# scitix/arks

Hardware: AMD Instinct MI355X
Metric: output_tok_s (higher is better)
Workload: dtype bf16; 1 GPU; model=qwen2.5-7b, global_batch=64, seq_len=1024, parallelism=dp1

## Files before the change

arks_amd/ops/__init__.py:

```python

from __future__ import annotations

import os
from typing import Callable, NamedTuple

import torch

from . import ref

_C = None
_C_ERR: str | None = None


def _load_extension():
    global _C, _C_ERR
    if _C is not None or _C_ERR is not None:
        return _C
    try:
        from . import _load

        _C = _load.C
    except Exception as e:
        _C_ERR = f"{type(e).__name__}: {e}"
    return _C
# ... 59 lines not shown
                   cos_sin, head_dim: int):
    if q.is_cuda:
        _native().rope_and_cache(positions, q, k, v, k_cache, v_cache,
                                 slot_mapping, cos_sin, head_dim)
        return q, k
    q2, k2 = ref.rope_apply(positions, q, k, cos_sin, head_dim)
    T = q.shape[0]
    nkv = k.numel() // max(T, 1) // head_dim
    ref.reshape_and_cache(
        k2.reshape(T, nkv, head_dim), v.reshape(T, nkv, head_dim),
        k_cache, v_cache, slot_mapping,
    )
    return q2, k2


def rope_and_cache_splitk(positions, qkv, k_cache, v_cache, slot_mapping,
                          cos_sin, head_dim: int, num_q_heads: int):
    qkv.check_live()
    if qkv.shape[1] != (num_q_heads + 2 * k_cache.shape[1]) * head_dim:
        raise ValueError(f"qkv width {qkv.shape[1]} does not match the heads")
    q = torch.empty((qkv.shape[0], num_q_heads * head_dim),
                    dtype=torch.bfloat16, device=qkv.ws.device)
    _native().splitk_rope_and_cache(positions, qkv.ws, qkv.bias, q, k_cache,
                                    v_cache, slot_mapping, cos_sin, head_dim,
                                    qkv.nsplits, qkv.mrows)
    return q


def reshape_and_cache(k, v, k_cache, v_cache, slot_mapping):
    if k.is_cuda:
        _native().reshape_and_cache(k, v, k_cache, v_cache, slot_mapping)
        return
    ref.reshape_and_cache(k, v, k_cache, v_cache, slot_mapping)


PREFILL_QTILE = 64


def build_prefill_tiles(seq_lens: list[int], device) -> torch.Tensor:
    tiles = []
# ... 207 lines not shown

    def materialize(self) -> torch.Tensor:
        self.check_live()
        out = torch.empty(self.shape, dtype=torch.bfloat16,
                          device=self.ws.device)
        _native().skinny_combine(out, self.ws, self.bias, self.nsplits,
                                 self.mrows)
        return out


def skinny_gemm(x, weight, bias=None, defer: bool = False):
    M, K = x.shape
    N = weight.shape[0]
    config, nsplits, k_per_split, mrows = _skinny_plan(M, N, K)
    config = _skinny_resident_config(config, M, nsplits, k_per_split)
    part = (_skinny_ws(nsplits, N, mrows, x.device) if nsplits > 1
            else x.new_empty(0, dtype=torch.float32))
    if defer and nsplits > 1:
        _native().skinny_gemm_partials(part, x, weight, k_per_split, nsplits,
                                       config)
        return SplitKPending(part, nsplits, mrows, M, N, bias,
                             (x.device.index,))
    out = torch.empty((M, N), dtype=x.dtype, device=x.device)
    _native().skinny_gemm(out, part, x, weight, bias, k_per_split, nsplits,
                          config)
    return out


def _skinny_plan(M: int, N: int, K: int):
    ntiles = N // 64
# ... 7 lines not shown
    nsplits = -(-K // k_per_split)
    return config, nsplits, k_per_split, 16 * mt


_SKINNY_RESIDENT_KMAX = 512
_SKINNY_RESIDENT = os.environ.get("ARKS_SKINNY_RESIDENT", "1") == "1"
_SKINNY_RESIDENT_MIN_M = 1


def _skinny_resident_config(config: int, M: int, nsplits: int,
                            k_per_split: int) -> int:
    if (_SKINNY_RESIDENT and config == 0 and nsplits > 1
            and k_per_split <= _SKINNY_RESIDENT_KMAX
            and M >= _SKINNY_RESIDENT_MIN_M):
        return 3
    return config


def _skinny_ws(nsplits: int, N: int, mrows: int, device):
    key = (device.index,)
    need = nsplits * N * mrows
    ws = _SKINNY_WS.get(key)
    if ws is None or ws.numel() < need:
        ws = torch.empty(need, dtype=torch.float32, device=device)
        _SKINNY_WS[key] = ws
    _SKINNY_WS_GEN[key] = _SKINNY_WS_GEN.get(key, 0) + 1
    return ws


_USE_SKINNY = os.environ.get("ARKS_SKINNY_GEMM", "1") == "1"
# ... 300 lines not shown
        out = torch.empty(T, H, dtype=y.dtype, device=y.device)
        _native().moe_mix(out, y.contiguous(), weights, ids, expert_base, El)
        return out
    return ref.moe_mix(y, weights, ids, expert_base)


def moe_mix_rows(y, weights, rows):
    if y.is_cuda:
        T, k = weights.shape
        out = torch.empty(T, y.shape[1], dtype=y.dtype, device=y.device)
        _native().moe_mix_rows(out, y.contiguous(), weights, rows)
        return out
    return ref.moe_mix_rows(y, weights, rows)


def sample_tokens(logits, temperatures, uniform):
    if logits.is_cuda:
        out = torch.empty(logits.shape[0], dtype=torch.int64, device=logits.device)
        _native().gumbel_sample(out, logits, temperatures, uniform)
        return out
    return ref.gumbel_sample(logits, temperatures, uniform)


def greedy_sample(logits):
    if logits.is_cuda:
        out = torch.empty(logits.shape[0], dtype=torch.int64, device=logits.device)
        _native().greedy_sample(out, logits)
        return out
    return ref.greedy_sample(logits)


def greedy_sample_masked(logits, masks, mask_row):
    if logits.is_cuda:
        out = torch.empty(logits.shape[0], dtype=torch.int64, device=logits.device)
        _native().greedy_sample_masked(out, logits, masks, mask_row)
        return out
    return ref.greedy_sample_masked(logits, masks, mask_row)


def sample_tokens_masked(logits, temperatures, uniform, masks, mask_row):
    if logits.is_cuda:
        out = torch.empty(logits.shape[0], dtype=torch.int64, device=logits.device)
        _native().gumbel_sample_masked(out, logits, temperatures, uniform,
# ... 114 lines not shown
```

arks_amd/ops/csrc/bindings.cpp:

```cpp
#include <torch/extension.h>

#include <c10/hip/HIPStream.h>
#include <hip/hip_runtime.h>

#include <cstring>
#include <string>
#include <vector>

namespace py = pybind11;

extern "C" {
void arks_rmsnorm(void* out, const void* input, const void* weight, float eps,
                  int rows, int hidden, hipStream_t stream);
void arks_fused_add_rmsnorm(void* out, const void* input, void* residual,
                            const void* weight, float eps, int rows, int hidden,
                            hipStream_t stream);
void arks_silu_mul(void* out, const void* gate_up, int64_t rows, int d,
                   hipStream_t stream);
int arks_pool_max_hidden();
void arks_pool_embed(void* out, void* carry, void* part, const void* x,
                     const void* residual, const void* weight,
                     const void* segs, const void* slabs, int nsegs,
                     int nslabs, float eps, int hidden, int dims,
                     int normalize, hipStream_t stream);
// ... 59 lines not shown
int arks_skinny_slab_rows(int m_rows, int config);
int arks_skinny_resident_kmax();
void arks_skinny_combine(void* out, const void* part, const void* bias,
                         int m_rows, int n_total, int nsplits, int mrows_pad,
                         hipStream_t stream);
void arks_splitk_add_rmsnorm(void* out, const void* part, const void* bias,
                             void* residual, const void* weight, float eps,
                             int rows, int hidden, int nsplits, int mrows_pad,
                             hipStream_t stream);
void arks_splitk_rope_and_cache(const void* positions, const void* part,
                                const void* bias, void* q_out, void* k_cache,
                                void* v_cache, const void* slot_mapping,
                                const void* cos_sin, int num_tokens,
                                int head_dim, int num_q_heads,
                                int num_kv_heads, int block_size, int nsplits,
                                int mrows_pad, int kv_fp8, hipStream_t stream);
void arks_greedy_sample(void* out, const void* logits, int rows, int vocab,
                        hipStream_t stream);
void arks_gumbel_sample(void* out, const void* logits, const void* temperatures,
                        const void* uniform, int rows, int vocab,
                        hipStream_t stream);
void arks_greedy_sample_masked(void* out, const void* logits,
                               const void* masks, const void* mask_row,
                               int rows, int vocab, int slots,
                               hipStream_t stream);
void arks_gumbel_sample_masked(void* out, const void* logits,
                               const void* temperatures, const void* uniform,
                               const void* masks, const void* mask_row,
                               int rows, int vocab, int slots,
                               hipStream_t stream);
void arks_apply_token_bitmask(void* logits, int is_fp32, const void* masks,
                              const void* mask_row, int rows, int vocab,
                              int slots, hipStream_t stream);
void arks_ar_seq_inc(void* seq, hipStream_t stream);
void arks_one_shot_allreduce(void* out, const void* src, void* mail_ptrs[8],
                             void* flag_ptrs[8], void* seq, int rank,
// ... 301 lines not shown
  TORCH_CHECK(combine_table.scalar_type() == torch::kInt32 &&
              combine_table.dim() == 2 && combine_table.size(1) == 4);
  const int num_q_heads = out.size(1);
  const int head_dim = out.size(2);
  arks_attn_extend2_combine(out.data_ptr(), part_ws.data_ptr(),
                            combine_table.data_ptr(), cu_seqlens_q.data_ptr(),
                            combine_table.size(0), (float)scale, num_q_heads,
                            head_dim, current_stream());
}

const void* check_skinny_args(const torch::Tensor& out,
                              const torch::Tensor& part,
                              const torch::Tensor& a, const torch::Tensor& w,
                              const c10::optional<torch::Tensor>& bias,
                              int64_t k, int64_t nsplits, int64_t mrows,
                              bool partials_only, const char* what) {
  check_bf16_rowstrided(a, "a");
  check_bf16_contig(w, "w");
  const int64_t m = a.size(0), n = w.size(0);
  TORCH_CHECK(m >= 1 && m <= 64, what, " needs 1 <= M <= 64");
  TORCH_CHECK(n % 64 == 0 && k % 32 == 0, "N%64==0 and K%32==0 required");
  if (partials_only) {
    TORCH_CHECK(nsplits > 1, what, ": partials-only needs nsplits > 1");
  } else {
    check_bf16_contig(out, "out");
    TORCH_CHECK(out.size(0) == m && out.size(1) == n);
  }
  const void* bias_ptr = nullptr;
  if (bias.has_value()) {
    check_bf16_contig(*bias, "bias");
    TORCH_CHECK(bias->numel() == n);
    bias_ptr = bias->data_ptr();
  }
  if (nsplits > 1) {
    TORCH_CHECK(part.is_cuda() && part.scalar_type() == torch::kFloat32 &&
                part.is_contiguous() &&
                part.numel() >= (int64_t)nsplits * n * mrows,
                what, " workspace too small");
  }
  return bias_ptr;
}

void skinny_gemm_impl(torch::Tensor out, torch::Tensor part, torch::Tensor a,
                      torch::Tensor w, c10::optional<torch::Tensor> bias,
                      int64_t k_per_split, int64_t nsplits, int64_t config,
                      int64_t groups, bool combine) {
  const int m = a.size(0), k = a.size(1), n = w.size(0);
  TORCH_CHECK(w.size(1) == k);
  TORCH_CHECK(0 <= config && config <= 3, "config in 0..3");
  TORCH_CHECK(k_per_split >= 32 && k_per_split % 32 == 0 &&
              nsplits * k_per_split >= k, "splits must cover K");
  TORCH_CHECK(config != 3 ||
                  (nsplits > 1 && k_per_split <= arks_skinny_resident_kmax()),
              "config 3 needs nsplits > 1 and k_per_split <= ",
              arks_skinny_resident_kmax());
  TORCH_CHECK(0 <= groups && groups <= 65535, "groups in 0..65535");
  TORCH_CHECK(nsplits <= 65535, "too many splits");
  const int mrows = arks_skinny_slab_rows(m, (int)config);
  const void* bias_ptr = check_skinny_args(out, part, a, w, bias, k, nsplits,
                                           mrows, !combine, "skinny_gemm");
  arks_skinny_gemm(nsplits > 1 ? part.data_ptr() : nullptr,
                   combine ? out.data_ptr() : nullptr, a.data_ptr(),
                   w.data_ptr(), bias_ptr, m, n, k, (int)k_per_split,
                   (int)nsplits, a.stride(0), (int)config, combine,
                   current_stream(), (int)groups);
}

void skinny_gemm(torch::Tensor out, torch::Tensor part, torch::Tensor a,
                 torch::Tensor w, c10::optional<torch::Tensor> bias,
                 int64_t k_per_split, int64_t nsplits, int64_t config,
                 int64_t groups) {
  skinny_gemm_impl(out, part, a, w, bias, k_per_split, nsplits, config, groups,
                   true);
}

// ... 277 lines not shown
              weight.numel() == hidden);
  const void* bias_ptr = check_partials(part, bias, nsplits, mrows, rows,
                                        hidden);
  if (rows == 0) return;
  arks_splitk_add_rmsnorm(out.data_ptr(), part.data_ptr(), bias_ptr,
                          residual.data_ptr(), weight.data_ptr(), (float)eps,
                          rows, hidden, (int)nsplits, (int)mrows,
                          current_stream());
}

void splitk_rope_and_cache(torch::Tensor positions, torch::Tensor part,
                           c10::optional<torch::Tensor> bias,
                           torch::Tensor q_out, torch::Tensor k_cache,
                           torch::Tensor v_cache, torch::Tensor slot_mapping,
                           torch::Tensor cos_sin, int64_t head_dim,
                           int64_t nsplits, int64_t mrows) {
  TORCH_CHECK(positions.scalar_type() == torch::kInt64 &&
              positions.is_contiguous());
  TORCH_CHECK(slot_mapping.scalar_type() == torch::kInt64 &&
              slot_mapping.is_contiguous());
  TORCH_CHECK(cos_sin.scalar_type() == torch::kFloat32 &&
              cos_sin.is_contiguous() && cos_sin.size(-1) == head_dim);
  check_bf16_contig(q_out, "q_out");
  const bool kv_fp8 = check_kv_cache(k_cache, "k_cache");
  TORCH_CHECK(check_kv_cache(v_cache, "v_cache") == kv_fp8);
  TORCH_CHECK(q_out.dim() == 2 && head_dim % 8 == 0);
  const int T = q_out.size(0);
  const int nq = (int)(q_out.size(1) / head_dim);
  const int nkv = k_cache.size(1);
  const int block_size = k_cache.size(2);
  TORCH_CHECK(nq * head_dim == q_out.size(1) && k_cache.size(3) == head_dim &&
              v_cache.sizes() == k_cache.sizes());
  TORCH_CHECK(positions.numel() == T && slot_mapping.numel() == T);
  const void* bias_ptr = check_partials(part, bias, nsplits, mrows, T,
                                        (int64_t)(nq + 2 * nkv) * head_dim);
  arks_splitk_rope_and_cache(positions.data_ptr(), part.data_ptr(), bias_ptr,
                             q_out.data_ptr(), k_cache.data_ptr(),
                             v_cache.data_ptr(), slot_mapping.data_ptr(),
                             cos_sin.data_ptr(), T, (int)head_dim, nq, nkv,
                             block_size, (int)nsplits, (int)mrows,
                             kv_fp8 ? 1 : 0, current_stream());
}

void rmsnorm_fp8(torch::Tensor out, torch::Tensor inv_scale,
                 torch::Tensor input, c10::optional<torch::Tensor> residual,
                 torch::Tensor weight, double eps) {
  check_bf16_contig(input, "input");
  check_bf16_contig(weight, "weight");
  TORCH_CHECK(out.scalar_type() == torch::kFloat8_e4m3fn && out.is_contiguous());
  TORCH_CHECK(inv_scale.scalar_type() == torch::kFloat32);
  const int hidden = input.size(-1);
  TORCH_CHECK(hidden % 8 == 0 && hidden <= 8192,
              "rmsnorm_fp8 requires hidden % 8 == 0 and hidden <= 8192");
  const int rows = input.numel() / hidden;
  void* res_ptr = nullptr;
  if (residual.has_value()) {
// ... 16 lines not shown
  const int rows = out.numel() / d;
  arks_silu_mul_fp8(out.data_ptr(), inv_scale.data_ptr(), gate_up.data_ptr(),
                    rows, d, current_stream());
}

void quant_fp8_rows(torch::Tensor out, torch::Tensor inv_scale,
                    torch::Tensor x) {
  check_bf16_contig(x, "x");
  TORCH_CHECK(out.scalar_type() == torch::kFloat8_e4m3fn && out.is_contiguous());
  TORCH_CHECK(inv_scale.scalar_type() == torch::kFloat32);
  TORCH_CHECK(x.size(1) % 8 == 0, "cols must be a multiple of 8");
  arks_quant_fp8_rows(out.data_ptr(), inv_scale.data_ptr(), x.data_ptr(),
                      x.size(0), x.size(1), current_stream());
}

void greedy_sample(torch::Tensor out, torch::Tensor logits) {
  check_bf16_contig(logits, "logits");
  TORCH_CHECK(out.scalar_type() == torch::kInt64);
  arks_greedy_sample(out.data_ptr(), logits.data_ptr(), logits.size(0),
                     logits.size(1), current_stream());
}

void gumbel_sample(torch::Tensor out, torch::Tensor logits,
                   torch::Tensor temperatures, torch::Tensor uniform) {
  check_bf16_contig(logits, "logits");
  TORCH_CHECK(out.scalar_type() == torch::kInt64);
  TORCH_CHECK(temperatures.scalar_type() == torch::kFloat32);
  TORCH_CHECK(uniform.scalar_type() == torch::kFloat32);
  arks_gumbel_sample(out.data_ptr(), logits.data_ptr(), temperatures.data_ptr(),
                     uniform.data_ptr(), logits.size(0), logits.size(1),
                     current_stream());
}

static void check_bitmask(const torch::Tensor& logits,
                          const torch::Tensor& masks,
                          const torch::Tensor& mask_row) {
  TORCH_CHECK(logits.dim() == 2 && masks.dim() == 2 && mask_row.dim() == 1);
  TORCH_CHECK(masks.is_cuda() && mask_row.is_cuda());
  TORCH_CHECK(masks.scalar_type() == torch::kInt32 && masks.is_contiguous());
  TORCH_CHECK(mask_row.scalar_type() == torch::kInt32 &&
              mask_row.is_contiguous());
  TORCH_CHECK(masks.size(1) == (logits.size(1) + 31) / 32,
              "masks must have ceil(vocab/32) words per row");
  TORCH_CHECK(mask_row.size(0) == logits.size(0), "one mask_row per row");
}
// ... 335 lines not shown
  m.def("skinny_gemm", &skinny_gemm, py::arg("out"), py::arg("part"),
        py::arg("a"), py::arg("w"), py::arg("bias"), py::arg("k_per_split"),
        py::arg("nsplits"), py::arg("config") = 0, py::arg("groups") = 0);
  m.def("skinny_gemm_partials", &skinny_gemm_partials, py::arg("part"),
        py::arg("a"), py::arg("w"), py::arg("k_per_split"),
        py::arg("nsplits"), py::arg("config") = 0, py::arg("groups") = 0);
  m.def("skinny_combine", &skinny_combine);
  m.def("w4_skinny_gemm", &w4_skinny_gemm);
  m.def("w4_skinny_gemm_partials", &w4_skinny_gemm_partials);
  m.def("w4_dequant", &w4_dequant);
  m.def("w4_moe_gemm", &w4_moe_gemm);
  m.def("w8_skinny_gemm", &w8_skinny_gemm);
  m.def("w8_skinny_gemm_partials", &w8_skinny_gemm_partials);
  m.def("w8_dequant", &w8_dequant);
  m.def("splitk_add_rmsnorm", &splitk_add_rmsnorm);
  m.def("splitk_rope_and_cache", &splitk_rope_and_cache);
  m.def("greedy_sample", &greedy_sample);
  m.def("gumbel_sample", &gumbel_sample);
  m.def("greedy_sample_masked", &greedy_sample_masked);
  m.def("gumbel_sample_masked", &gumbel_sample_masked);
  m.def("apply_token_bitmask", &apply_token_bitmask);
  m.def("ipc_alloc", &ipc_alloc);
  m.def("arm_flags", &arm_flags);
  m.def("ipc_alloc_free", &ipc_alloc_free);
  m.def("ipc_handle", &ipc_handle);
  m.def("ipc_open", &ipc_open);
  m.def("ipc_close", &ipc_close);
  m.def("one_shot_allreduce", &one_shot_allreduce);
  m.def("moe_topk", &moe_topk);
  m.def("moe_route", &moe_route);
  m.def("moe_mix", &moe_mix);
  m.def("moe_mix_rows", &moe_mix_rows);
  m.def("lora_shrink", &lora_shrink);
// ... 7 lines not shown
```

arks_amd/ops/csrc/kvcache.hip:

```cpp
#include "kv_store.h"

#include <type_traits>

namespace arks {

template <bool FP8>
__global__ void reshape_and_cache_kernel(
    const bf16* __restrict__ k,
    const bf16* __restrict__ v,
    void* __restrict__ k_cache,
    void* __restrict__ v_cache,
    const int64_t* __restrict__ slot_mapping,
    const int num_kv_heads, const int head_dim, const int block_size,
    const int64_t kv_stride) {
  const int token = blockIdx.x;
  const CachePage pg =
      cache_page(slot_mapping[token], num_kv_heads, block_size, head_dim);
  if (!pg.valid) return;
  const int nvec = num_kv_heads * head_dim / 8;
  const bf16* k_src = k + (int64_t)token * kv_stride;
  const bf16* v_src = v + (int64_t)token * kv_stride;
  for (int i = threadIdx.x; i < nvec; i += blockDim.x) {
    const int h = (i * 8) / head_dim;
    const int d = (i * 8) % head_dim;
// ... 78 lines not shown
    const int block_size, const int nsplits, const int64_t split_stride) {
  const int token = blockIdx.x;
  const int half = head_dim / 2;
  const int n_total = (num_q_heads + 2 * num_kv_heads) * head_dim;
  const int64_t pos = positions[token];
  const float* cs = cos_sin + pos * head_dim;
  const CachePage pg =
      cache_page(slot_mapping[token], num_kv_heads, block_size, head_dim);
  const float* part_row = part + (int64_t)token * n_total;

  const int quads = half / 4;
  const int nrot_q = num_q_heads * quads;
  const int nrot = pg.valid ? nrot_q + num_kv_heads * quads : nrot_q;
  const int nvec = pg.valid ? num_kv_heads * head_dim / 8 : 0;
  const int v_col0 = (num_q_heads + num_kv_heads) * head_dim;
  for (int idx = threadIdx.x; idx < nrot + nvec; idx += blockDim.x) {
    if (idx < nrot) {
      const int h = idx / quads;
      const int p4 = (idx % quads) * 4;
      const int col = h * head_dim + p4;
      const float* const p[2] = {part_row + col, part_row + col + half};
      float4v acc[2];
      splitk_reduce<2, 1>(p, split_stride, nsplits, acc);
      ushort4v o1, o2;
#pragma unroll
      for (int j = 0; j < 4; ++j) {
        float af = acc[0][j];
        float bf = acc[1][j];
        if (bias != nullptr) {
          af += bf16_bits_to_float(bias[col + j]);
          bf += bf16_bits_to_float(bias[col + half + j]);
// ... 56 lines not shown
  int threads = std::min(256, num_kv_heads * head_dim / 8);
  dispatch_kv_fp8(kv_fp8, [&](auto fp8) {
    hipLaunchKernelGGL((reshape_and_cache_kernel<decltype(fp8)::value>),
                       dim3(num_tokens), dim3(threads), 0, stream,
                       (const bf16*)k, (const bf16*)v, k_cache, v_cache,
                       (const int64_t*)slot_mapping, num_kv_heads, head_dim,
                       block_size, kv_stride);
  });
}

extern "C" void arks_splitk_rope_and_cache(
    const void* positions, const void* part, const void* bias, void* q_out,
    void* k_cache, void* v_cache, const void* slot_mapping,
    const void* cos_sin, int num_tokens, int head_dim, int num_q_heads,
    int num_kv_heads, int block_size, int nsplits, int mrows_pad, int kv_fp8,
    hipStream_t stream) {
  if (num_tokens == 0) return;
  const int items = (num_q_heads + num_kv_heads) * (head_dim / 8) +
                    num_kv_heads * head_dim / 8;
  dim3 grid(num_tokens), block(std::min(1024, (items + 63) / 64 * 64));
  const int64_t split_stride =
      (int64_t)mrows_pad * (num_q_heads + 2 * num_kv_heads) * head_dim;
  dispatch_kv_fp8(kv_fp8, [&](auto fp8) {
    hipLaunchKernelGGL((splitk_rope_cache_kernel<decltype(fp8)::value>), grid,
                       block, 0, stream, (const int64_t*)positions,
                       (const float*)part, (const bf16*)bias, (bf16*)q_out,
                       k_cache, v_cache, (const int64_t*)slot_mapping,
                       (const float*)cos_sin, head_dim, num_q_heads,
                       num_kv_heads, block_size, nsplits, split_stride);
  });
}

extern "C" void arks_rope_and_cache(
    const void* positions, void* q, void* k, const void* v, void* k_cache,
    void* v_cache, const void* slot_mapping, const void* cos_sin,
// ... 15 lines not shown
```

arks_amd/ops/csrc/sampling.hip:

```cpp
#include "common.h"

#include <cfloat>

namespace arks {

template <bool GUMBEL>
__global__ void sample_kernel(int64_t* __restrict__ out,
                              const bf16* __restrict__ logits,
                              const float* __restrict__ temperatures,
                              const float* __restrict__ uniform,
                              const int vocab) {
  constexpr int BLOCK = 256;
  const int row = blockIdx.x;
  const bf16* lrow = logits + (int64_t)row * vocab;
  float inv_t = 0.f;
  bool greedy = true;
  if constexpr (GUMBEL) {
    const float t = temperatures[row];
    greedy = (t <= 0.f);
    inv_t = greedy ? 1.f : 1.f / t;
  }
  const float* urow = GUMBEL ? uniform + (int64_t)row * vocab : nullptr;

  float best = -FLT_MAX;
  int best_idx = 0;
  const int nvec = vocab / 8;
  for (int i = threadIdx.x; i < nvec; i += BLOCK) {
    ushort8 x = *reinterpret_cast<const ushort8*>(lrow + i * 8);
#pragma unroll
    for (int j = 0; j < 8; ++j) {
      float v = bf16_bits_to_float(x[j]);
      if constexpr (GUMBEL) {
        if (!greedy) {
          float u = urow[i * 8 + j];
          u = fmaxf(u, 1e-20f);
          v = v * inv_t - __logf(-__logf(u));
        }
      }
      const int idx = i * 8 + j;
      if (v > best || (v == best && idx < best_idx)) {
        best = v;
        best_idx = idx;
      }
    }
  }
  for (int idx = nvec * 8 + threadIdx.x; idx < vocab; idx += BLOCK) {
    float v = bf16_bits_to_float(lrow[idx]);
    if constexpr (GUMBEL) {
      if (!greedy) {
        float u = fmaxf(urow[idx], 1e-20f);
        v = v * inv_t - __logf(-__logf(u));
      }
    }
    if (v > best || (v == best && idx < best_idx)) {
      best = v;
      best_idx = idx;
    }
  }

#pragma unroll
  for (int off = 32; off > 0; off >>= 1) {
    float ov = __shfl_xor(best, off, WAVE_SIZE);
    int oi = __shfl_xor(best_idx, off, WAVE_SIZE);
    if (ov > best || (ov == best && oi < best_idx)) {
      best = ov;
      best_idx = oi;
    }
  }
  __shared__ float sval[BLOCK / WAVE_SIZE];
  __shared__ int sidx[BLOCK / WAVE_SIZE];
  const int wave = threadIdx.x / WAVE_SIZE;
  if (threadIdx.x % WAVE_SIZE == 0) {
    sval[wave] = best;
    sidx[wave] = best_idx;
  }
  __syncthreads();
  if (threadIdx.x == 0) {
    float b = sval[0];
    int bi = sidx[0];
#pragma unroll
    for (int w = 1; w < BLOCK / WAVE_SIZE; ++w) {
      if (sval[w] > b || (sval[w] == b && sidx[w] < bi)) {
        b = sval[w];
        bi = sidx[w];
      }
    }
    out[row] = bi;
  }
}

constexpr int NO_TOKEN = 0x7fffffff;

__device__ __forceinline__ void masked_take(float v, int idx, float& best,
                                            int& best_idx, bool allowed = true) {
  const bool take =
      allowed & ((v > best) | ((v == best) & (idx < best_idx)));
  best = take ? v : best;
  best_idx = take ? idx : best_idx;
}

template <bool GUMBEL>
__global__ void sample_masked_kernel(int64_t* __restrict__ out,
                                     const bf16* __restrict__ logits,
// ... 115 lines not shown
  if (idx0 >= vocab) return;
  const uint32_t word = masks[(int64_t)mr * words + (idx0 >> 5)];
  const uint32_t bits = (word >> (idx0 & 31)) & 0xffu;
  if (bits == 0xffu) return;
  T* lrow = logits + (int64_t)row * vocab;
#pragma unroll
  for (int j = 0; j < 8; ++j) {
    if (idx0 + j < vocab && !((bits >> j) & 1u)) lrow[idx0 + j] = neg_inf;
  }
}

}

using namespace arks;

extern "C" {

void arks_greedy_sample_masked(void* out, const void* logits,
                               const void* masks, const void* mask_row,
                               int rows, int vocab, int slots,
                               hipStream_t stream) {
  hipLaunchKernelGGL((sample_masked_kernel<false>), dim3(rows), dim3(256), 0,
                     stream, (int64_t*)out, (const bf16*)logits, nullptr,
                     nullptr, (const uint32_t*)masks, (const int*)mask_row,
                     vocab, (vocab + 31) / 32, slots);
}

void arks_gumbel_sample_masked(void* out, const void* logits,
                               const void* temperatures, const void* uniform,
                               const void* masks, const void* mask_row,
// ... 11 lines not shown
                              int slots, hipStream_t stream) {
  const dim3 grid(rows, (vocab + 2047) / 2048);
  const int words = (vocab + 31) / 32;
  if (is_fp32) {
    hipLaunchKernelGGL((apply_bitmask_kernel<float>), grid, dim3(256), 0,
                       stream, (float*)logits, (const uint32_t*)masks,
                       (const int*)mask_row, vocab, words, slots, -INFINITY);
  } else {
    hipLaunchKernelGGL((apply_bitmask_kernel<uint16_t>), grid, dim3(256), 0,
                       stream, (uint16_t*)logits, (const uint32_t*)masks,
                       (const int*)mask_row, vocab, words, slots,
                       (uint16_t)0xff80);
  }
}

void arks_greedy_sample(void* out, const void* logits, int rows, int vocab,
                        hipStream_t stream) {
  hipLaunchKernelGGL((sample_kernel<false>), dim3(rows), dim3(256), 0, stream,
                     (int64_t*)out, (const bf16*)logits, nullptr, nullptr,
                     vocab);
}

void arks_gumbel_sample(void* out, const void* logits, const void* temperatures,
                        const void* uniform, int rows, int vocab,
                        hipStream_t stream) {
  hipLaunchKernelGGL((sample_kernel<true>), dim3(rows), dim3(256), 0, stream,
                     (int64_t*)out, (const bf16*)logits,
                     (const float*)temperatures, (const float*)uniform, vocab);
}

}
```

arks_amd/ops/csrc/skinny_gemm.hip:

```cpp
#include "common.h"

#include <algorithm>
#include <atomic>
#include <cfloat>
#include <type_traits>

namespace arks {

typedef __attribute__((ext_vector_type(8))) __bf16 bf16x8;
typedef __attribute__((ext_vector_type(4))) float f32x4;

__device__ __forceinline__ f32x4 sk_mfma(bf16x8 a, bf16x8 b, f32x4 c) {
  return __builtin_amdgcn_mfma_f32_16x16x32_bf16(a, b, c, 0, 0, 0);
}

constexpr int SK_AP = 8;

template <int MT>
__device__ __forceinline__ void store_partials(float* __restrict__ part,
                                               const f32x4 (&acc)[MT],
                                               const int n_total,
                                               const int n, const int lq) {
  float* p = part + (int64_t)blockIdx.y * (16 * MT) * n_total + n;
#pragma unroll
// ... 8 lines not shown
__global__ __launch_bounds__(64 * WAVES, 2) void skinny_gemm_kernel(
    float* __restrict__ part,
    bf16* __restrict__ out,
    const bf16* __restrict__ a,
    const bf16* __restrict__ w,
    const bf16* __restrict__ bias,
    const int m_rows, const int n_total, const int k_total,
    const int k_per_split, const int nsplits, const int64_t a_stride) {
  constexpr int KC = SK_KC;
  constexpr int D = SK_D;
  constexpr int KSTEPS = KC / 32;
  constexpr int CPT = KC / 8;
  constexpr int THREADS = 64 * WAVES;
  constexpr int NTW = 16 * WAVES;
  constexpr int RPP = THREADS / CPT;
  constexpr int NIT = 16 * MT / RPP;
  static_assert(D % 2 == 0, "LDS slot parity follows the ring slot");
  static_assert(NIT * RPP == 16 * MT, "A chunk must divide over the threads");
  const int n0 = blockIdx.x * NTW;
  const int kb = blockIdx.y * k_per_split;
  const int ke = min(k_total, kb + k_per_split);
  const int klen = max(ke - kb, 0);
  const int nch = (klen + KC - 1) / KC;

  const int tid = threadIdx.x;
  const int wave = tid / WAVE_SIZE;
  const int lane = tid % WAVE_SIZE;
  const int lq = lane % 16;
  const int la = lane / 16;

  __shared__ __attribute__((aligned(16))) union {
    bf16 a_buf[2][64][KC + SK_AP];
    float c_buf[NTW][64 + 1];
// ... 25 lines not shown
      ad[it] = *reinterpret_cast<const ushort8*>(live ? src : a);
    }
#pragma unroll
    for (int s = 0; s < KSTEPS; ++s) {
      const bf16* wsrc = wrow + min(kc + s * 32, k_total - 32);
      const ushort8* src =
          reinterpret_cast<const ushort8*>(live ? wsrc : w);
      if constexpr (NT)
        wd[s] = __builtin_nontemporal_load(src);
      else
        wd[s] = *src;
    }
  };
  auto write_a = [&](const ushort8 (&ad)[NIT], int buf) {
#pragma unroll
    for (int it = 0; it < NIT; ++it)
      *reinterpret_cast<ushort8*>(
          &lds.a_buf[buf][tid / CPT + it * RPP][acol]) = ad[it];
  };
  auto mfma_chunk = [&](const ushort8 (&wd)[KSTEPS], int buf, int kw) {
#pragma unroll
    for (int s = 0; s < KSTEPS; ++s) {
      if (s * 32 >= kw) break;
      ushort8 wv = wd[s];
      bf16x8 wfrag = *reinterpret_cast<bf16x8*>(&wv);
#pragma unroll
      for (int t = 0; t < MT; ++t) {
        ushort8 af = *reinterpret_cast<const ushort8*>(
            &lds.a_buf[buf][t * 16 + lq][s * 32 + 8 * la]);
        acc[t] = sk_mfma(wfrag, *reinterpret_cast<bf16x8*>(&af), acc[t]);
      }
    }
  };
// ... 315 lines not shown
      launch_resident<decltype(mt)::value>(
          (float*)part, (const bf16*)a, (const bf16*)w, m_rows, n_total,
          k_total, k_per_split, nsplits, a_stride, groups, stream);
    };
    switch (skinny_mt(m_rows, config)) {
      case 1: launch(std::integral_constant<int, 1>{}); break;
      case 2: launch(std::integral_constant<int, 2>{}); break;
      case 3: launch(std::integral_constant<int, 3>{}); break;
      default: launch(std::integral_constant<int, 4>{}); break;
    }
    if (combine)
      arks_skinny_combine(out, part, bias, m_rows, n_total, nsplits,
                          arks_skinny_slab_rows(m_rows, config), stream);
    return;
  }
  const int waves = config == 0 ? 4 : 8;
  dim3 grid((n_total + 16 * waves - 1) / (16 * waves), nsplits);
  dim3 block(64 * waves);
  auto launch = [&](auto kernel) {
    hipLaunchKernelGGL(kernel, grid, block, 0, stream, (float*)part,
                       (bf16*)out, (const bf16*)a, (const bf16*)w,
                       (const bf16*)bias, m_rows, n_total, k_total,
                       k_per_split, nsplits, a_stride);
  };
  if (config == 2) {
    launch(skinny_gemm_kernel<4, true, 8>);
  } else if (config == 1) {
    launch(skinny_gemm_kernel<4, false, 8>);
  } else {
    switch (skinny_mt(m_rows, config)) {
      case 1: launch(skinny_gemm_kernel<1>); break;
      case 2: launch(skinny_gemm_kernel<2>); break;
      case 3: launch(skinny_gemm_kernel<3>); break;
      default: launch(skinny_gemm_kernel<4>); break;
    }
  }
  if (nsplits > 1 && combine)
    arks_skinny_combine(out, part, bias, m_rows, n_total, nsplits,
                        arks_skinny_slab_rows(m_rows, config), stream);
}
// ... 1 lines not shown
```

Before: 12140 tok/s.

## Split sampling, rope-cache and tall-K skinny GEMM across more workgroups

Adds a chunked two-pass argmax sampler that splits each vocab row over several workgroups when rows are fewer than CUs, then merges per-chunk pairs. Also splits the split-K rope/KV-cache kernel over a second grid dimension sized from the CU count. Adds a 7-wave (112-column) tall-K skinny GEMM variant, chosen when it fills more CUs without exceeding them. The aim is better CU occupancy for small-batch decode, at the cost of an extra merge launch and workspace allocation.

```diff
diff --git a/arks_amd/ops/__init__.py b/arks_amd/ops/__init__.py
--- a/arks_amd/ops/__init__.py
+++ b/arks_amd/ops/__init__.py
@@ -97,16 +97,28 @@
     return q2, k2
 
 
+_ROPE_SPLITK_GROUPS = int(os.environ.get("ARKS_ROPE_SPLITK_GROUPS", "0"))
+
+
+def _rope_splitk_groups(tokens: int, cus: int) -> int:
+    if _ROPE_SPLITK_GROUPS > 0:
+        return _ROPE_SPLITK_GROUPS
+    return max(1, -(-cus // max(tokens, 1)))
+
+
 def rope_and_cache_splitk(positions, qkv, k_cache, v_cache, slot_mapping,
-                          cos_sin, head_dim: int, num_q_heads: int):
+                          cos_sin, head_dim: int, num_q_heads: int,
+                          groups: int | None = None):
     qkv.check_live()
     if qkv.shape[1] != (num_q_heads + 2 * k_cache.shape[1]) * head_dim:
         raise ValueError(f"qkv width {qkv.shape[1]} does not match the heads")
     q = torch.empty((qkv.shape[0], num_q_heads * head_dim),
                     dtype=torch.bfloat16, device=qkv.ws.device)
+    if groups is None:
+        groups = _rope_splitk_groups(qkv.shape[0], _cu_count(qkv.ws.device))
     _native().splitk_rope_and_cache(positions, qkv.ws, qkv.bias, q, k_cache,
                                     v_cache, slot_mapping, cos_sin, head_dim,
-                                    qkv.nsplits, qkv.mrows)
+                                    qkv.nsplits, qkv.mrows, groups)
     return q
 
 
@@ -344,6 +356,9 @@
     N = weight.shape[0]
     config, nsplits, k_per_split, mrows = _skinny_plan(M, N, K)
     config = _skinny_resident_config(config, M, nsplits, k_per_split)
+    if config == 1:
+        config = _skinny_tallk7_config(config, N, nsplits,
+                                       _cu_count(x.device))
     part = (_skinny_ws(nsplits, N, mrows, x.device) if nsplits > 1
             else x.new_empty(0, dtype=torch.float32))
     if defer and nsplits > 1:
@@ -381,6 +396,23 @@
             and k_per_split <= _SKINNY_RESIDENT_KMAX
             and M >= _SKINNY_RESIDENT_MIN_M):
         return 3
+    return config
+
+
+_TALLK_WAVES = os.environ.get("ARKS_SKINNY_TALLK_WAVES", "7").strip()
+if _TALLK_WAVES not in ("7", "8"):
+    raise ValueError(
+        f"ARKS_SKINNY_TALLK_WAVES={_TALLK_WAVES!r}: accepted values are 7 "
+        "(112-row tiles where they fill more CUs) and 8 (128-row tiles)"
+    )
+
+
+def _skinny_tallk7_config(config: int, N: int, nsplits: int, cus: int) -> int:
+    if _TALLK_WAVES != "7" or config != 1 or N % 112 != 0:
+        return config
+    wgs = N // 112 * nsplits
+    if wgs <= cus and wgs > -(-N // 128) * nsplits:
+        return 4
     return config
 
 
@@ -711,19 +743,49 @@
     return ref.moe_mix_rows(y, weights, rows)
 
 
-def sample_tokens(logits, temperatures, uniform):
+_CU_COUNT: dict = {}
+
+
+def _cu_count(device) -> int:
+    idx = device.index if device.index is not None else torch.cuda.current_device()
+    n = _CU_COUNT.get(idx)
+    if n is None:
+        n = _CU_COUNT[idx] = torch.cuda.get_device_properties(idx).multi_processor_count
+    return n
+
+
+_SAMPLE_MIN_CHUNK = 2048
+_SAMPLE_WGS_PER_CU = 4
+
+
+def _sample_chunks(rows: int, vocab: int, cus: int) -> int:
+    if rows >= cus:
+        return 1
+    want = -(-_SAMPLE_WGS_PER_CU * cus // max(rows, 1))
+    return max(1, min(want, vocab // _SAMPLE_MIN_CHUNK))
+
+
+def _sample_launch(fn, logits, args, chunks):
+    rows, vocab = logits.shape
+    if chunks is None:
+        chunks = _sample_chunks(rows, vocab, _cu_count(logits.device))
+    out = torch.empty(rows, dtype=torch.int64, device=logits.device)
+    pairs = (torch.empty((rows, chunks, 2), dtype=torch.int32,
+                         device=logits.device) if chunks > 1 else None)
+    fn(out, logits, *args, pairs, chunks)
+    return out
+
+
+def sample_tokens(logits, temperatures, uniform, chunks=None):
     if logits.is_cuda:
-        out = torch.empty(logits.shape[0], dtype=torch.int64, device=logits.device)
-        _native().gumbel_sample(out, logits, temperatures, uniform)
-        return out
+        return _sample_launch(_native().gumbel_sample, logits,
+                              (temperatures, uniform), chunks)
     return ref.gumbel_sample(logits, temperatures, uniform)
 
 
-def greedy_sample(logits):
+def greedy_sample(logits, chunks=None):
     if logits.is_cuda:
-        out = torch.empty(logits.shape[0], dtype=torch.int64, device=logits.device)
-        _native().greedy_sample(out, logits)
-        return out
+        return _sample_launch(_native().greedy_sample, logits, (), chunks)
     return ref.greedy_sample(logits)
 
 
diff --git a/arks_amd/ops/csrc/bindings.cpp b/arks_amd/ops/csrc/bindings.cpp
--- a/arks_amd/ops/csrc/bindings.cpp
+++ b/arks_amd/ops/csrc/bindings.cpp
@@ -97,12 +97,13 @@
                                 const void* cos_sin, int num_tokens,
                                 int head_dim, int num_q_heads,
                                 int num_kv_heads, int block_size, int nsplits,
-                                int mrows_pad, int kv_fp8, hipStream_t stream);
-void arks_greedy_sample(void* out, const void* logits, int rows, int vocab,
-                        hipStream_t stream);
-void arks_gumbel_sample(void* out, const void* logits, const void* temperatures,
-                        const void* uniform, int rows, int vocab,
-                        hipStream_t stream);
+                                int mrows_pad, int kv_fp8, int groups,
+                                hipStream_t stream);
+void arks_greedy_sample(void* out, void* pairs, const void* logits, int rows,
+                        int vocab, int chunks, hipStream_t stream);
+void arks_gumbel_sample(void* out, void* pairs, const void* logits,
+                        const void* temperatures, const void* uniform,
+                        int rows, int vocab, int chunks, hipStream_t stream);
 void arks_greedy_sample_masked(void* out, const void* logits,
                                const void* masks, const void* mask_row,
                                int rows, int vocab, int slots,
@@ -434,12 +435,14 @@
                               const torch::Tensor& a, const torch::Tensor& w,
                               const c10::optional<torch::Tensor>& bias,
                               int64_t k, int64_t nsplits, int64_t mrows,
-                              bool partials_only, const char* what) {
+                              int64_t n_mult, bool partials_only,
+                              const char* what) {
   check_bf16_rowstrided(a, "a");
   check_bf16_contig(w, "w");
   const int64_t m = a.size(0), n = w.size(0);
   TORCH_CHECK(m >= 1 && m <= 64, what, " needs 1 <= M <= 64");
-  TORCH_CHECK(n % 64 == 0 && k % 32 == 0, "N%64==0 and K%32==0 required");
+  TORCH_CHECK(n % n_mult == 0 && k % 32 == 0, "N%", n_mult,
+              "==0 and K%32==0 required");
   if (partials_only) {
     TORCH_CHECK(nsplits > 1, what, ": partials-only needs nsplits > 1");
   } else {
@@ -467,7 +470,7 @@
                       int64_t groups, bool combine) {
   const int m = a.size(0), k = a.size(1), n = w.size(0);
   TORCH_CHECK(w.size(1) == k);
-  TORCH_CHECK(0 <= config && config <= 3, "config in 0..3");
+  TORCH_CHECK(0 <= config && config <= 4, "config in 0..4");
   TORCH_CHECK(k_per_split >= 32 && k_per_split % 32 == 0 &&
               nsplits * k_per_split >= k, "splits must cover K");
   TORCH_CHECK(config != 3 ||
@@ -477,8 +480,10 @@
   TORCH_CHECK(0 <= groups && groups <= 65535, "groups in 0..65535");
   TORCH_CHECK(nsplits <= 65535, "too many splits");
   const int mrows = arks_skinny_slab_rows(m, (int)config);
-  const void* bias_ptr = check_skinny_args(out, part, a, w, bias, k, nsplits,
-                                           mrows, !combine, "skinny_gemm");
+  const void* bias_ptr =
+      check_skinny_args(out, part, a, w, bias, k, nsplits, mrows,
+                        config == 0 || config == 3 ? 64 : 16, !combine,
+                        "skinny_gemm");
   arks_skinny_gemm(nsplits > 1 ? part.data_ptr() : nullptr,
                    combine ? out.data_ptr() : nullptr, a.data_ptr(),
                    w.data_ptr(), bias_ptr, m, n, k, (int)k_per_split,
@@ -786,7 +791,8 @@
                            torch::Tensor q_out, torch::Tensor k_cache,
                            torch::Tensor v_cache, torch::Tensor slot_mapping,
                            torch::Tensor cos_sin, int64_t head_dim,
-                           int64_t nsplits, int64_t mrows) {
+                           int64_t nsplits, int64_t mrows, int64_t groups) {
+  TORCH_CHECK(1 <= groups && groups <= 65535, "groups in 1..65535");
   TORCH_CHECK(positions.scalar_type() == torch::kInt64 &&
               positions.is_contiguous());
   TORCH_CHECK(slot_mapping.scalar_type() == torch::kInt64 &&
@@ -811,7 +817,7 @@
                              v_cache.data_ptr(), slot_mapping.data_ptr(),
                              cos_sin.data_ptr(), T, (int)head_dim, nq, nkv,
                              block_size, (int)nsplits, (int)mrows,
-                             kv_fp8 ? 1 : 0, current_stream());
+                             kv_fp8 ? 1 : 0, (int)groups, current_stream());
 }
 
 void rmsnorm_fp8(torch::Tensor out, torch::Tensor inv_scale,
@@ -858,21 +864,40 @@
                       x.size(0), x.size(1), current_stream());
 }
 
-void greedy_sample(torch::Tensor out, torch::Tensor logits) {
+static void* check_sample_pairs(const torch::Tensor& out,
+                                const torch::Tensor& logits,
+                                const c10::optional<torch::Tensor>& pairs,
+                                int64_t chunks) {
   check_bf16_contig(logits, "logits");
-  TORCH_CHECK(out.scalar_type() == torch::kInt64);
-  arks_greedy_sample(out.data_ptr(), logits.data_ptr(), logits.size(0),
-                     logits.size(1), current_stream());
+  TORCH_CHECK(logits.dim() == 2);
+  TORCH_CHECK(out.scalar_type() == torch::kInt64 && out.is_contiguous() &&
+              out.numel() >= logits.size(0));
+  TORCH_CHECK(1 <= chunks && chunks <= 65535, "chunks in 1..65535");
+  if (chunks == 1) return nullptr;
+  TORCH_CHECK(pairs.has_value() && pairs->is_cuda() &&
+                  pairs->scalar_type() == torch::kInt32 &&
+                  pairs->is_contiguous() &&
+                  pairs->numel() >= logits.size(0) * chunks * 2,
+              "chunks > 1 needs an int32 workspace of rows * chunks * 2");
+  return pairs->data_ptr();
+}
+
+void greedy_sample(torch::Tensor out, torch::Tensor logits,
+                   c10::optional<torch::Tensor> pairs, int64_t chunks) {
+  void* ws = check_sample_pairs(out, logits, pairs, chunks);
+  arks_greedy_sample(out.data_ptr(), ws, logits.data_ptr(), logits.size(0),
+                     logits.size(1), (int)chunks, current_stream());
 }
 
 void gumbel_sample(torch::Tensor out, torch::Tensor logits,
-                   torch::Tensor temperatures, torch::Tensor uniform) {
-  check_bf16_contig(logits, "logits");
-  TORCH_CHECK(out.scalar_type() == torch::kInt64);
+                   torch::Tensor temperatures, torch::Tensor uniform,
+                   c10::optional<torch::Tensor> pairs, int64_t chunks) {
+  void* ws = check_sample_pairs(out, logits, pairs, chunks);
   TORCH_CHECK(temperatures.scalar_type() == torch::kFloat32);
   TORCH_CHECK(uniform.scalar_type() == torch::kFloat32);
-  arks_gumbel_sample(out.data_ptr(), logits.data_ptr(), temperatures.data_ptr(),
-                     uniform.data_ptr(), logits.size(0), logits.size(1),
+  arks_gumbel_sample(out.data_ptr(), ws, logits.data_ptr(),
+                     temperatures.data_ptr(), uniform.data_ptr(),
+                     logits.size(0), logits.size(1), (int)chunks,
                      current_stream());
 }
 
@@ -1238,9 +1263,16 @@
   m.def("w8_skinny_gemm_partials", &w8_skinny_gemm_partials);
   m.def("w8_dequant", &w8_dequant);
   m.def("splitk_add_rmsnorm", &splitk_add_rmsnorm);
-  m.def("splitk_rope_and_cache", &splitk_rope_and_cache);
-  m.def("greedy_sample", &greedy_sample);
-  m.def("gumbel_sample", &gumbel_sample);
+  m.def("splitk_rope_and_cache", &splitk_rope_and_cache, py::arg("positions"),
+        py::arg("part"), py::arg("bias"), py::arg("q_out"), py::arg("k_cache"),
+        py::arg("v_cache"), py::arg("slot_mapping"), py::arg("cos_sin"),
+        py::arg("head_dim"), py::arg("nsplits"), py::arg("mrows"),
+        py::arg("groups") = 1);
+  m.def("greedy_sample", &greedy_sample, py::arg("out"), py::arg("logits"),
+        py::arg("pairs") = py::none(), py::arg("chunks") = 1);
+  m.def("gumbel_sample", &gumbel_sample, py::arg("out"), py::arg("logits"),
+        py::arg("temperatures"), py::arg("uniform"),
+        py::arg("pairs") = py::none(), py::arg("chunks") = 1);
   m.def("greedy_sample_masked", &greedy_sample_masked);
   m.def("gumbel_sample_masked", &gumbel_sample_masked);
   m.def("apply_token_bitmask", &apply_token_bitmask);
diff --git a/arks_amd/ops/csrc/kvcache.hip b/arks_amd/ops/csrc/kvcache.hip
--- a/arks_amd/ops/csrc/kvcache.hip
+++ b/arks_amd/ops/csrc/kvcache.hip
@@ -116,7 +116,8 @@
   const int nrot = pg.valid ? nrot_q + num_kv_heads * quads : nrot_q;
   const int nvec = pg.valid ? num_kv_heads * head_dim / 8 : 0;
   const int v_col0 = (num_q_heads + num_kv_heads) * head_dim;
-  for (int idx = threadIdx.x; idx < nrot + nvec; idx += blockDim.x) {
+  for (int idx = blockIdx.y * blockDim.x + threadIdx.x; idx < nrot + nvec;
+       idx += blockDim.x * gridDim.y) {
     if (idx < nrot) {
       const int h = idx / quads;
       const int p4 = (idx % quads) * 4;
@@ -203,11 +204,14 @@
     void* k_cache, void* v_cache, const void* slot_mapping,
     const void* cos_sin, int num_tokens, int head_dim, int num_q_heads,
     int num_kv_heads, int block_size, int nsplits, int mrows_pad, int kv_fp8,
-    hipStream_t stream) {
+    int groups, hipStream_t stream) {
   if (num_tokens == 0) return;
   const int items = (num_q_heads + num_kv_heads) * (head_dim / 8) +
                     num_kv_heads * head_dim / 8;
-  dim3 grid(num_tokens), block(std::min(1024, (items + 63) / 64 * 64));
+  groups = std::max(1, std::min(groups, (items + 63) / 64));
+  const int per_group = (items + groups - 1) / groups;
+  dim3 grid(num_tokens, groups);
+  dim3 block(std::min(1024, (per_group + 63) / 64 * 64));
   const int64_t split_stride =
       (int64_t)mrows_pad * (num_q_heads + 2 * num_kv_heads) * head_dim;
   dispatch_kv_fp8(kv_fp8, [&](auto fp8) {
diff --git a/arks_amd/ops/csrc/sampling.hip b/arks_amd/ops/csrc/sampling.hip
--- a/arks_amd/ops/csrc/sampling.hip
+++ b/arks_amd/ops/csrc/sampling.hip
@@ -1,31 +1,33 @@
 #include "common.h"
 
+#include <algorithm>
 #include <cfloat>
 
 namespace arks {
 
+constexpr int SAMPLE_BLOCK = 256;
+
+__device__ __forceinline__ void sample_take(float v, int idx, float& best,
+                                            int& best_idx) {
+  if (v > best || (v == best && idx < best_idx)) {
+    best = v;
+    best_idx = idx;
+  }
+}
+
 template <bool GUMBEL>
-__global__ void sample_kernel(int64_t* __restrict__ out,
-                              const bf16* __restrict__ logits,
-                              const float* __restrict__ temperatures,
-                              const float* __restrict__ uniform,
-                              const int vocab) {
-  constexpr int BLOCK = 256;
-  const int row = blockIdx.x;
-  const bf16* lrow = logits + (int64_t)row * vocab;
-  float inv_t = 0.f;
-  bool greedy = true;
-  if constexpr (GUMBEL) {
-    const float t = temperatures[row];
-    greedy = (t <= 0.f);
-    inv_t = greedy ? 1.f : 1.f / t;
-  }
-  const float* urow = GUMBEL ? uniform + (int64_t)row * vocab : nullptr;
-
-  float best = -FLT_MAX;
-  int best_idx = 0;
-  const int nvec = vocab / 8;
-  for (int i = threadIdx.x; i < nvec; i += BLOCK) {
+__device__ __forceinline__ bool sample_scan(const bf16* __restrict__ lrow,
+                                            const float* __restrict__ urow,
+                                            const bool greedy,
+                                            const float inv_t, const int begin,
+                                            const int end, float& best,
+                                            int& best_idx) {
+  constexpr int BLOCK = SAMPLE_BLOCK;
+  best = -FLT_MAX;
+  best_idx = 0;
+  const int vec0 = begin / 8;
+  const int nvec = end / 8;
+  for (int i = vec0 + threadIdx.x; i < nvec; i += BLOCK) {
     ushort8 x = *reinterpret_cast<const ushort8*>(lrow + i * 8);
 #pragma unroll
     for (int j = 0; j < 8; ++j) {
@@ -37,14 +39,10 @@
           v = v * inv_t - __logf(-__logf(u));
         }
       }
-      const int idx = i * 8 + j;
-      if (v > best || (v == best && idx < best_idx)) {
-        best = v;
-        best_idx = idx;
-      }
-    }
-  }
-  for (int idx = nvec * 8 + threadIdx.x; idx < vocab; idx += BLOCK) {
+      sample_take(v, i * 8 + j, best, best_idx);
+    }
+  }
+  for (int idx = nvec * 8 + threadIdx.x; idx < end; idx += BLOCK) {
     float v = bf16_bits_to_float(lrow[idx]);
     if constexpr (GUMBEL) {
       if (!greedy) {
@@ -52,20 +50,14 @@
         v = v * inv_t - __logf(-__logf(u));
       }
     }
-    if (v > best || (v == best && idx < best_idx)) {
-      best = v;
-      best_idx = idx;
-    }
+    sample_take(v, idx, best, best_idx);
   }
 
 #pragma unroll
   for (int off = 32; off > 0; off >>= 1) {
     float ov = __shfl_xor(best, off, WAVE_SIZE);
     int oi = __shfl_xor(best_idx, off, WAVE_SIZE);
-    if (ov > best || (ov == best && oi < best_idx)) {
-      best = ov;
-      best_idx = oi;
-    }
+    sample_take(ov, oi, best, best_idx);
   }
   __shared__ float sval[BLOCK / WAVE_SIZE];
   __shared__ int sidx[BLOCK / WAVE_SIZE];
@@ -75,18 +67,67 @@
     sidx[wave] = best_idx;
   }
   __syncthreads();
-  if (threadIdx.x == 0) {
-    float b = sval[0];
-    int bi = sidx[0];
-#pragma unroll
-    for (int w = 1; w < BLOCK / WAVE_SIZE; ++w) {
-      if (sval[w] > b || (sval[w] == b && sidx[w] < bi)) {
-        b = sval[w];
-        bi = sidx[w];
-      }
-    }
-    out[row] = bi;
-  }
+  if (threadIdx.x != 0) return false;
+  best = sval[0];
+  best_idx = sidx[0];
+#pragma unroll
+  for (int w = 1; w < BLOCK / WAVE_SIZE; ++w)
+    sample_take(sval[w], sidx[w], best, best_idx);
+  return true;
+}
+
+template <bool GUMBEL>
+__global__ __launch_bounds__(SAMPLE_BLOCK) void sample_kernel(
+    int64_t* __restrict__ out,
+    int2* __restrict__ pairs,
+    const bf16* __restrict__ logits,
+    const float* __restrict__ temperatures,
+    const float* __restrict__ uniform,
+    const int vocab, const int chunk_len) {
+  const int row = blockIdx.x;
+  const bf16* lrow = logits + (int64_t)row * vocab;
+  float inv_t = 0.f;
+  bool greedy = true;
+  if constexpr (GUMBEL) {
+    const float t = temperatures[row];
+    greedy = (t <= 0.f);
+    inv_t = greedy ? 1.f : 1.f / t;
+  }
+  const float* urow = GUMBEL ? uniform + (int64_t)row * vocab : nullptr;
+
+  const int begin =
+      (int)std::min<int64_t>((int64_t)blockIdx.y * chunk_len, vocab);
+  const int end = (int)std::min<int64_t>((int64_t)begin + chunk_len, vocab);
+  float best;
+  int best_idx;
+  if (!sample_scan<GUMBEL>(lrow, urow, greedy, inv_t, begin, end, best,
+                           best_idx))
+    return;
+  if (gridDim.y == 1)
+    out[row] = best_idx;
+  else
+    pairs[(int64_t)row * gridDim.y + blockIdx.y] =
+        make_int2(__float_as_int(best), best_idx);
+}
+
+__global__ __launch_bounds__(64) void sample_merge_kernel(
+    int64_t* __restrict__ out, const int2* __restrict__ pairs, const int rows,
+    const int chunks) {
+  const int row = blockIdx.x * 64 + threadIdx.x;
+  if (row >= rows) return;
+  float best = -FLT_MAX;
+  int best_idx = 0;
+  constexpr int BATCH = 16;
+  const int2* prow = pairs + (int64_t)row * chunks;
+  for (int c = 0; c < chunks; c += BATCH) {
+    int2 p[BATCH];
+#pragma unroll
+    for (int j = 0; j < BATCH; ++j) p[j] = prow[min(c + j, chunks - 1)];
+#pragma unroll
+    for (int j = 0; j < BATCH; ++j)
+      sample_take(__int_as_float(p[j].x), p[j].y, best, best_idx);
+  }
+  out[row] = best_idx;
 }
 
 constexpr int NO_TOKEN = 0x7fffffff;
@@ -232,6 +273,25 @@
 
 using namespace arks;
 
+template <bool GUMBEL>
+static void launch_sample(void* out, void* pairs, const void* logits,
+                          const void* temperatures, const void* uniform,
+                          int rows, int vocab, int chunks,
+                          hipStream_t stream) {
+  chunks = std::max(chunks, 1);
+  const int chunk_len =
+      chunks == 1 ? vocab : ((vocab + chunks - 1) / chunks + 7) / 8 * 8;
+  hipLaunchKernelGGL((sample_kernel<GUMBEL>), dim3(rows, chunks),
+                     dim3(SAMPLE_BLOCK), 0, stream, (int64_t*)out,
+                     (int2*)pairs, (const bf16*)logits,
+                     (const float*)temperatures, (const float*)uniform, vocab,
+                     chunk_len);
+  if (chunks > 1)
+    hipLaunchKernelGGL(sample_merge_kernel, dim3((rows + 63) / 64), dim3(64),
+                       0, stream, (int64_t*)out, (const int2*)pairs, rows,
+                       chunks);
+}
+
 extern "C" {
 
 void arks_greedy_sample_masked(void* out, const void* logits,
@@ -273,19 +333,17 @@
   }
 }
 
-void arks_greedy_sample(void* out, const void* logits, int rows, int vocab,
-                        hipStream_t stream) {
-  hipLaunchKernelGGL((sample_kernel<false>), dim3(rows), dim3(256), 0, stream,
-                     (int64_t*)out, (const bf16*)logits, nullptr, nullptr,
-                     vocab);
-}
-
-void arks_gumbel_sample(void* out, const void* logits, const void* temperatures,
-                        const void* uniform, int rows, int vocab,
-                        hipStream_t stream) {
-  hipLaunchKernelGGL((sample_kernel<true>), dim3(rows), dim3(256), 0, stream,
-                     (int64_t*)out, (const bf16*)logits,
-                     (const float*)temperatures, (const float*)uniform, vocab);
-}
-
-}
+void arks_greedy_sample(void* out, void* pairs, const void* logits, int rows,
+                        int vocab, int chunks, hipStream_t stream) {
+  launch_sample<false>(out, pairs, logits, nullptr, nullptr, rows, vocab,
+                       chunks, stream);
+}
+
+void arks_gumbel_sample(void* out, void* pairs, const void* logits,
+                        const void* temperatures, const void* uniform,
+                        int rows, int vocab, int chunks, hipStream_t stream) {
+  launch_sample<true>(out, pairs, logits, temperatures, uniform, rows, vocab,
+                      chunks, stream);
+}
+
+}
diff --git a/arks_amd/ops/csrc/skinny_gemm.hip b/arks_amd/ops/csrc/skinny_gemm.hip
--- a/arks_amd/ops/csrc/skinny_gemm.hip
+++ b/arks_amd/ops/csrc/skinny_gemm.hip
@@ -46,9 +46,8 @@
   constexpr int THREADS = 64 * WAVES;
   constexpr int NTW = 16 * WAVES;
   constexpr int RPP = THREADS / CPT;
-  constexpr int NIT = 16 * MT / RPP;
+  constexpr int NIT = (16 * MT + RPP - 1) / RPP;
   static_assert(D % 2 == 0, "LDS slot parity follows the ring slot");
-  static_assert(NIT * RPP == 16 * MT, "A chunk must divide over the threads");
   const int n0 = blockIdx.x * NTW;
   const int kb = blockIdx.y * k_per_split;
   const int ke = min(k_total, kb + k_per_split);
@@ -104,9 +103,11 @@
   };
   auto write_a = [&](const ushort8 (&ad)[NIT], int buf) {
 #pragma unroll
-    for (int it = 0; it < NIT; ++it)
-      *reinterpret_cast<ushort8*>(
-          &lds.a_buf[buf][tid / CPT + it * RPP][acol]) = ad[it];
+    for (int it = 0; it < NIT; ++it) {
+      int row = tid / CPT + it * RPP;
+      if constexpr (NIT * RPP != 16 * MT) row = min(row, 16 * MT - 1);
+      *reinterpret_cast<ushort8*>(&lds.a_buf[buf][row][acol]) = ad[it];
+    }
   };
   auto mfma_chunk = [&](const ushort8 (&wd)[KSTEPS], int buf, int kw) {
 #pragma unroll
@@ -452,7 +453,7 @@
                           arks_skinny_slab_rows(m_rows, config), stream);
     return;
   }
-  const int waves = config == 0 ? 4 : 8;
+  const int waves = config == 0 ? 4 : config == 4 ? 7 : 8;
   dim3 grid((n_total + 16 * waves - 1) / (16 * waves), nsplits);
   dim3 block(64 * waves);
   auto launch = [&](auto kernel) {
@@ -461,7 +462,9 @@
                        (const bf16*)bias, m_rows, n_total, k_total,
                        k_per_split, nsplits, a_stride);
   };
-  if (config == 2) {
+  if (config == 4) {
+    launch(skinny_gemm_kernel<4, false, 7>);
+  } else if (config == 2) {
     launch(skinny_gemm_kernel<4, true, 8>);
   } else if (config == 1) {
     launch(skinny_gemm_kernel<4, false, 8>);
```

After: 12460 tok/s (median of 6 runs). 1.03x the previous value.
